# OpenResearchInstitute/ka9q-sdr

Hardware: AMD Instinct MI355X
Metric: input Msamples/s + channels @ real-time, 16384-pt overlap-save (higher is better)
Workload: dtype f32

## Files before the change

ka9q_sdr_amd/csrc/kq_pruned.hip:

```cpp
#include <cstdlib>
#include <type_traits>

#include "kq_device.hpp"
#include "kq_lane.hpp"
#include "kq_regfft.hpp"

namespace kq {

namespace {

__device__ __forceinline__ rfft::v2f as_v2f(float2 a) { return (rfft::v2f){a.x, a.y}; }
__device__ __forceinline__ float2 as_f2(rfft::v2f a) { return make_float2(a.x, a.y); }
__device__ __forceinline__ float2 cmul(float2 a, float2 b) { return as_f2(rfft::pk_cmul(as_v2f(a), as_v2f(b))); }
__device__ __forceinline__ float2 cmulc(float2 a, float2 b) { return as_f2(rfft::pk_cmul_any(as_v2f(a), as_v2f(b))); }
__device__ __forceinline__ float2 cadd(float2 a, float2 b) { return make_float2(a.x + b.x, a.y + b.y); }
__device__ __forceinline__ float2 csub(float2 a, float2 b) { return make_float2(a.x - b.x, a.y - b.y); }
__device__ __forceinline__ float2 cconj(float2 a) { return make_float2(a.x, -a.y); }
__device__ __forceinline__ float2 cfma_v(float2 b, float2 c, float2 a) { return as_f2(rfft::pk_cmadd(as_v2f(b), as_v2f(c), as_v2f(a))); }
__device__ __forceinline__ float2 cfma(float2 b, float2 c, float2 a) {
  rfft::v2f const bb = as_v2f(b), cc = as_v2f(c);
  return as_f2(rfft::pk_fma((rfft::v2f){-bb.y, bb.y}, cc.yx, rfft::pk_fma(bb.xx, cc, as_v2f(a))));
}

using rfft::bitrev5;
using rfft::kPi;
using rfft::tw_im;
using rfft::tw_re;
__device__ __forceinline__ void fft32_dit(float2 (&v)[32]) {
  rfft::v2f w[32];
#pragma unroll
  for (int i = 0; i < 32; i++) w[i] = as_v2f(v[i]);
  rfft::fft_dit_pk<32>(w);
#pragma unroll
  for (int i = 0; i < 32; i++) v[i] = as_f2(w[i]);
}

template <int ND>
struct Tab {
  static constexpr int P = ND / 32;
  static constexpr int kA = (ND == 64) ? 2 * 32 * 4 : (ND == 128) ? 32 * P * 2 : P * 32 * P * 2;
  static constexpr int kT = ND * 2;
  static constexpr int kL = 6 * ND * 2;
  static constexpr int kFloats = kA + kT + kL;
  static constexpr int kWaveF4 = (ND == 256) ? ND / 2 : (kA + kT) / 4;
};

template <int ND>
__device__ __forceinline__ int signed_bin(int q) {
  return q <= ND / 2 ? q : q - ND;
}

template <int ND>
__device__ __forceinline__ float2 table_entry_AT(int i, double f, double r, int R, int N) {
  constexpr int P = ND / 32;
  constexpr int nA = Tab<ND>::kA / 2;
  if (i < nA) {
    double a, extra = 0;
    if (ND == 64) {
      int const pass = i >> 6, ap = (i >> 1) & 31, hf = i & 1;
      a = ap + 32 * hf;
      if (pass) extra = -(double)ap / 64.0 + (hf ? 0.5 : 0.0);
    } else if (ND == 128) {
      int const ap = i / P, s = i % P;
      a = ap + 32 * s;
    } else {
      int const pass = i / (32 * P), ap = (i / P) % 32, s = i % P;
      a = ap + 32 * s;
      extra = -(double)(s * pass) / 8.0 - (double)(ap * pass) / 256.0;
    }
    double const Ra = (double)R * a;
    return phasor_turns(f * Ra + r * (0.5 * Ra * (Ra - 1.0)) + extra);
  }
  int const t = i - nA;
  int const p = t >> 5, qp = t & 31;
  int const q = P * qp + p;
  double turns = 64.0 * f;
  turns -= rint(turns);
  turns -= 64.0 * (double)signed_bin<ND>(q) / (double)N;
  return phasor_turns(turns);
}

__device__ __forceinline__ void swap32(float &a, float &b) {
  auto const r = __builtin_amdgcn_permlane32_swap(__float_as_uint(a), __float_as_uint(b), false, false);
  a = __uint_as_float(r[0]);
  b = __uint_as_float(r[1]);
}

__device__ __forceinline__ void swap16(float &a, float &b) {
  auto const r = __builtin_amdgcn_permlane16_swap(__float_as_uint(a), __float_as_uint(b), false, false);
  a = __uint_as_float(r[0]);
  b = __uint_as_float(r[1]);
}
template <int I>
__device__ __forceinline__ void pair_dpp(float &e, float &o) {
  static_assert(I == 3 || I == 2, "lane bits 3 and 2: whole banks of four lanes");
  int const ei = __float_as_int(e), oi = __float_as_int(o);
  int lo, up;
  if constexpr (I == 3) {
    lo = __builtin_amdgcn_update_dpp(ei, oi, 0x128, 0xF, 0xC, false);
    up = __builtin_amdgcn_update_dpp(oi, ei, 0x128, 0xF, 0x3, false);
  } else {
    lo = __builtin_amdgcn_update_dpp(ei, oi, 0x114, 0xF, 0xA, false);
    up = __builtin_amdgcn_update_dpp(oi, ei, 0x104, 0xF, 0x5, false);
  }
  e = __int_as_float(lo);
  o = __int_as_float(up);
}

template <int ND, int PASS, int STRIDE, bool SWEPT>
__device__ __forceinline__ void column_pass(const float2 *col, const float4 *tab, const float2 *wsh, float kappa,
                                            float2 (&v)[32]) {
  constexpr int P = ND / 32;
  constexpr int CH = (ND == 64) ? 4 : (ND == 128) ? 2 : 1;
  constexpr int TW4 = (ND == 64) ? 1 : P / 2;
  float2 xs[2][CH][P];
  float4 tw[2][CH][TW4];
#pragma unroll
  for (int i = 0; i < CH; i++) {
#pragma unroll
    for (int s = 0; s < P; s++) xs[0][i][s] = col[STRIDE * (i + 32 * s)];
#pragma unroll
    for (int t = 0; t < TW4; t++) tw[0][i][t] = (ND == 64) ? tab[PASS * 32 + i] : tab[TW4 * i + t];
  }
#pragma unroll
  for (int k = 0; k < 32 / CH; k++) {
    int const cur = k & 1, nxt = cur ^ 1;
    if (k + 1 < 32 / CH) {
#pragma unroll
      for (int i = 0; i < CH; i++) {
        int const ap = (k + 1) * CH + i;
#pragma unroll
        for (int s = 0; s < P; s++) xs[nxt][i][s] = col[STRIDE * (ap + 32 * s)];
#pragma unroll
        for (int t = 0; t < TW4; t++) tw[nxt][i][t] = (ND == 64) ? tab[PASS * 32 + ap] : tab[TW4 * ap + t];
      }
    }
    __builtin_amdgcn_sched_barrier(0);
#pragma unroll
    for (int i = 0; i < CH; i++) {
      int const ap = k * CH + i;
      float2 x[P];
#pragma unroll
      for (int s = 0; s < P; s++) {
        x[s] = xs[cur][i][s];
        if (SWEPT) {
          float const ph = kappa * (float)(ap + 32 * s);
          x[s] = make_float2(fmaf(-ph, x[s].y, x[s].x), fmaf(ph, x[s].x, x[s].y));
        }
      }
      float2 r;
      if (ND == 64) {
        float4 const t = tw[cur][i][0];
        r = make_float2(x[0].x * t.x - x[0].y * t.y, x[0].x * t.y + x[0].y * t.x);
        r.x = fmaf(x[1].x, t.z, fmaf(-x[1].y, t.w, r.x));
        r.y = fmaf(x[1].x, t.w, fmaf(x[1].y, t.z, r.y));
      } else {
        float2 re = make_float2(0.f, 0.f), ro = make_float2(0.f, 0.f);
        bool first_e = true, first_o = true;
#pragma unroll
        for (int s = 0; s < P; s++) {
          float4 const t4 = tw[cur][i][s >> 1];
          float2 const A = (s & 1) ? make_float2(t4.z, t4.w) : make_float2(t4.x, t4.y);
          int const e8 = ((8 / P) * s * PASS) & 7;
          int const rot = e8 >> 1;
          float2 const As = rot == 0   ? A
                            : rot == 1 ? make_float2(A.y, -A.x)
                            : rot == 2 ? make_float2(-A.x, -A.y)
                                       : make_float2(-A.y, A.x);
          if (e8 & 1) {
            ro = first_o ? cmulc(x[s], As) : cfma(x[s], As, ro);
            first_o = false;
          } else {
            re = first_e ? cmulc(x[s], As) : cfma(x[s], As, re);
            first_e = false;
          }
        }
        r = re;
        if (!first_o) {
          float const h = 0.70710678118654752440f;
          r.x += (ro.x + ro.y) * h;
          r.y += (ro.y - ro.x) * h;
        }
        if (PASS != 0 && ap != 0) {
          r = cmul(r, wsh[(ap * PASS) % ND]);
        }
      }
      v[bitrev5(ap)] = r;
    }
    __builtin_amdgcn_sched_barrier(0);
  }
  fft32_dit(v);
  __builtin_amdgcn_sched_barrier(0);
}

__device__ __forceinline__ void horner(float2 (&acc)[32], const float2 (&v)[32], const float4 *tT) {
#pragma unroll
  for (int k = 0; k < 4; k++) {
    float4 w4[4];
#pragma unroll
    for (int i = 0; i < 4; i++) w4[i] = tT[k * 4 + i];
#pragma unroll
    for (int i = 0; i < 4; i++) {
      int const q0 = k * 8 + 2 * i;
      acc[q0] = cfma(make_float2(w4[i].x, w4[i].y), acc[q0], v[q0]);
      acc[q0 + 1] = cfma(make_float2(w4[i].z, w4[i].w), acc[q0 + 1], v[q0 + 1]);
    }
    __builtin_amdgcn_sched_barrier(0);
  }
}

template <int ND, int PASS, bool SWEPT>
__device__ __forceinline__ float2 lane_reduce(float2 (&acc)[32], const float2 *tL, const float2 (&th)[6], int lane) {
  constexpr int P = ND / 32;
  float2 z[16];
  int qlow;
  {
    int const bit = (lane >> 5) & 1;
    qlow = bit;
    const float2 *tl = tL + 5 * ND;
#pragma unroll
    for (int m = 0; m < 16; m++) {
      float2 e = acc[2 * m], o = acc[2 * m + 1];
      swap32(e.x, o.x);
      swap32(e.y, o.y);
      float2 w = tl[P * (2 * m + bit) + PASS];
      if (SWEPT) w = cmul(w, th[5]);
      z[m] = cfma_v(w, o, e);
    }
  }
#pragma unroll
  for (int t = 1; t < 5; t++) {
    int const i = 5 - t;
    int const bit = (lane >> i) & 1;
    int const cnt = 16 >> t;
    const float2 *tl = tL + (size_t)i * ND;
#pragma unroll
    for (int m = 0; m < cnt; m++) {
      float2 lo, hi;
      if (i >= 2) {
        lo = z[2 * m];
        hi = z[2 * m + 1];
        if (i == 4) {
          swap16(lo.x, hi.x);
          swap16(lo.y, hi.y);
        } else if (i == 3) {
          pair_dpp<3>(lo.x, hi.x);
          pair_dpp<3>(lo.y, hi.y);
        } else {
          pair_dpp<2>(lo.x, hi.x);
          pair_dpp<2>(lo.y, hi.y);
        }
      } else {
        float2 const e = z[2 * m], o = z[2 * m + 1];
        float2 const keep = bit ? o : e, send = bit ? e : o;
        float2 recv;
        recv.x = __shfl_xor(send.x, 1 << i, 64);
        recv.y = __shfl_xor(send.y, 1 << i, 64);
        lo = bit ? recv : keep;
        hi = bit ? keep : recv;
      }
      int const qp = (((2 * m + bit) << t) | qlow);
      float2 w = tl[P * qp + PASS];
      if (SWEPT) w = cmul(w, th[i]);
      z[m] = cfma_v(w, hi, lo);
    }
    qlow |= bit << t;
  }
  float2 recv;
  recv.x = __shfl_xor(z[0].x, 1, 64);
  recv.y = __shfl_xor(z[0].y, 1, 64);
  int const b0 = lane & 1;
  float2 const lo = b0 ? recv : z[0], hi = b0 ? z[0] : recv;
  float2 w = tL[P * qlow + PASS];
  if (SWEPT) w = cmul(w, th[0]);
  return cfma_v(w, hi, lo);
}

template <int ND>
__device__ __forceinline__ float2 lane_reduce_rt(float2 (&acc)[32], const float2 *tL, int pass, int lane) {
  constexpr int P = ND / 32;
  float2 z[16];
  int qlow;
  {
    int const bit = (lane >> 5) & 1;
    qlow = bit;
    const float2 *tl = tL + 5 * ND + pass;
#pragma unroll
    for (int m = 0; m < 16; m++) {
      float2 e = acc[2 * m], o = acc[2 * m + 1];
      swap32(e.x, o.x);
      swap32(e.y, o.y);
      z[m] = cfma_v(tl[P * (2 * m + bit)], o, e);
    }
  }
#pragma unroll
  for (int t = 1; t < 5; t++) {
    int const i = 5 - t;
    int const bit = (lane >> i) & 1;
    int const cnt = 16 >> t;
    const float2 *tl = tL + (size_t)i * ND + pass;
#pragma unroll
    for (int m = 0; m < cnt; m++) {
      float2 lo, hi;
      if (i >= 2) {
        lo = z[2 * m];
        hi = z[2 * m + 1];
        if (i == 4) {
          swap16(lo.x, hi.x);
          swap16(lo.y, hi.y);
        } else if (i == 3) {
          pair_dpp<3>(lo.x, hi.x);
          pair_dpp<3>(lo.y, hi.y);
        } else {
          pair_dpp<2>(lo.x, hi.x);
          pair_dpp<2>(lo.y, hi.y);
        }
      } else {
        float2 const e = z[2 * m], o = z[2 * m + 1];
        float2 const keep = bit ? o : e, send = bit ? e : o;
        float2 recv;
        recv.x = __shfl_xor(send.x, 1 << i, 64);
        recv.y = __shfl_xor(send.y, 1 << i, 64);
        lo = bit ? recv : keep;
        hi = bit ? keep : recv;
      }
      int const qp = (((2 * m + bit) << t) | qlow);
      z[m] = cfma_v(tl[P * qp], hi, lo);
    }
    qlow |= bit << t;
  }
  float2 recv;
  recv.x = __shfl_xor(z[0].x, 1, 64);
  recv.y = __shfl_xor(z[0].y, 1, 64);
  int const b0 = lane & 1;
  float2 const lo = b0 ? recv : z[0], hi = b0 ? z[0] : recv;
  return cfma_v(tL[P * qlow + pass], hi, lo);
}

template <int ND, bool SWEPT>
__device__ __forceinline__ void fill_tables(float4 *wtab, const float *tc, double f_blk, double df, double r, int R, int N,
                                            float2 (&th)[6], int lane) {
  if (SWEPT) {
    float2 *w2 = reinterpret_cast<float2 *>(wtab);
    for (int i = lane; i < Tab<ND>::kWaveF4 * 2; i += 64) w2[i] = table_entry_AT<ND>(i, f_blk, r, R, N);
#pragma unroll
    for (int i = 0; i < 6; i++) th[i] = phasor_turns((double)(1 << i) * df);
  } else {
    const float4 *src = reinterpret_cast<const float4 *>(tc);
    for (int i = lane; i < Tab<ND>::kWaveF4; i += 64) wtab[i] = src[i];
#pragma unroll
    for (int i = 0; i < 6; i++) th[i] = make_float2(1.f, 0.f);
  }
  wave_sync();
}

template <int ND>
__device__ __forceinline__ void epilogue_from_scratch(const float2 *scratch, bool isb, float2 *out, int olen, int lane);

template <int ND>
__device__ __forceinline__ void epilogue_lds(float2 *scratch, const float2 (&ypass)[ND / 32], float2 p0, const float2 *H,
                                             bool isb, float2 *out, int olen, int lane) {
  constexpr int P = ND / 32, V = ND / 64;
  int const b0 = lane & 1;
  int const qp = (int)(__brev((unsigned)(lane >> 1)) >> 27);
#pragma unroll
  for (int i = 0; i < V; i++) {
    float2 const y = b0 ? ypass[2 * i + 1] : ypass[2 * i];
    int const q = P * qp + 2 * i + b0;
    scratch[q] = cmul(cmul(y, p0), H[q]);
  }
  wave_sync();
  epilogue_from_scratch<ND>(scratch, isb, out, olen, lane);
}

template <int ND>
__device__ __forceinline__ void epilogue_from_scratch(const float2 *scratch, bool isb, float2 *out, int olen, int lane) {
  constexpr int V = ND / 64;
  constexpr int LOGN = (ND == 128) ? 7 : 8, LOGV = (ND == 128) ? 1 : 2;
  float2 z[V];
#pragma unroll
  for (int e = 0; e < V; e++) {
    int const q = (int)(__brev((unsigned)(V * lane + e)) >> (32 - LOGN));
    float2 gq = scratch[q];
    if (isb && q != 0 && q != ND / 2) {
      float2 const o = scratch[ND - q];
      gq = (q < ND / 2) ? cadd(gq, cconj(o)) : csub(gq, cconj(o));
    }
    z[e] = gq;
  }
#pragma unroll
  for (int s = 0; s < LOGV; s++) {
    int const half = 1 << s;
#pragma unroll
    for (int e = 0; e < V; e++) {
      if (e & half) continue;
      int const jj = e & (half - 1);
      float2 const a = z[e];
      float2 b = z[e + half];
      if (jj != 0) b = make_float2(-b.y, b.x);
      z[e] = cadd(a, b);
      z[e + half] = csub(a, b);
    }
  }
#pragma unroll
  for (int s = LOGV; s < LOGN; s++) {
    int const half = 1 << s;
    int const bit = (lane >> (s - LOGV)) & 1;
#pragma unroll
    for (int e = 0; e < V; e++) {
      int const jj = (V * lane + e) & (half - 1);
      float sw, cw;
      sincospif((float)jj / (float)half, &sw, &cw);
      float2 const v = bit ? cmul(z[e], make_float2(cw, sw)) : z[e];
      float2 rr;
      rr.x = __shfl_xor(v.x, half / V, 64);
      rr.y = __shfl_xor(v.y, half / V, 64);
      z[e] = bit ? csub(rr, v) : cadd(v, rr);
    }
  }
  int const first = ND - olen;
#pragma unroll
  for (int e = 0; e < V; e++) {
    int const pos = V * lane + e;
    if (pos >= first) out[pos - first] = z[e];
  }
}

}

template <int ND>
__global__ void k_pruned_tables(Geom g, ChanDev ch, float *__restrict__ tab, int nchan) {
  int const c = blockIdx.x;
  if (c >= nchan) return;
  double const f = ch.lo_freq[c];
  float2 *t = reinterpret_cast<float2 *>(tab + (size_t)c * Tab<ND>::kFloats);
  constexpr int nAT = (Tab<ND>::kA + Tab<ND>::kT) / 2;
  for (int i = threadIdx.x; i < nAT; i += blockDim.x) t[i] = table_entry_AT<ND>(i, f, 0.0, g.D, g.N);
  for (int i = threadIdx.x; i < 6 * ND; i += blockDim.x) {
    int const lvl = i / ND, q = i % ND;
    double const off = (double)(1 << lvl);
    double turns = off * f;
    turns -= rint(turns);
    turns -= off * (double)signed_bin<ND>(q) / (double)g.N;
    t[nAT + i] = phasor_turns(turns);
  }
}

template <int NWAVES, int CPW, int R, bool SWEPT>
__global__ void __launch_bounds__(NWAVES * 64) k_pruned_resident(Geom g, ChanDev ch, Planes pl,
                                                                 const float2 *__restrict__ window,
                                                                 const float *__restrict__ tab, int nchan,
                                                                 const int *__restrict__ chan_list, IirArgs iir) {
  constexpr int ND = 64;
  constexpr int N = ND * R;
  constexpr int groups = R / 64;
  extern __shared__ __attribute__((aligned(16))) float2 lds[];
  int const blk = blockIdx.y;
  {
    const float4 *src = reinterpret_cast<const float4 *>(window + (size_t)blk * g.L);
    float4 *dst = reinterpret_cast<float4 *>(lds);
    for (int i = threadIdx.x; i < N / 2; i += NWAVES * 64) dst[i] = src[i];
  }
  float2 *itw = lds + N + NWAVES * Tab<ND>::kWaveF4 * 2;
  if (threadIdx.x < 32) {
    float sw, cw;
    sincospif((float)threadIdx.x / 32.f, &sw, &cw);
    itw[threadIdx.x] = make_float2(cw, sw);
  }
  __syncthreads();
  int const wave = threadIdx.x >> 6, lane = threadIdx.x & 63;
  float4 *wtab = reinterpret_cast<float4 *>(lds + N) + wave * Tab<ND>::kWaveF4;
  int const b0 = lane & 1;
  double const m0 = (double)blk * g.L;

  for (int ci = 0; ci < CPW; ci++) {
    int const idx = __builtin_amdgcn_readfirstlane((blockIdx.x * NWAVES + wave) * CPW + ci);
    if (idx >= nchan) break;
    int const c = chan_list ? __builtin_amdgcn_readfirstlane(chan_list[idx]) : idx;
    const float *tc = tab + (size_t)c * Tab<ND>::kFloats;
    const float2 *tL = reinterpret_cast<const float2 *>(tc + Tab<ND>::kA + Tab<ND>::kT);
    double const f0 = ch.lo_freq[c], r = SWEPT ? ch.lo_rate[c] : 0.0;
    double const f_blk = f0 + r * m0;
    float2 th[6];
    fill_tables<ND, SWEPT>(wtab, tc, f_blk, r * m0, r, R, N, th, lane);
    const float4 *wT = wtab + Tab<ND>::kA / 4;
    float const kap_lane = SWEPT ? (float)(2.0 * kPi * r * (double)R) : 0.f;

    float2 y_even = make_float2(0.f, 0.f), y_odd = make_float2(0.f, 0.f);
#pragma unroll
    for (int pass = 0; pass < 2; pass++) {
      float2 acc[32];
#pragma unroll 1
      for (int j = groups - 1; j >= 0; j--) {
        const float2 *col = lds + 64 * j + lane;
        float const kappa = kap_lane * (float)(64 * j + lane);
        float2 v[32];
        if (pass == 0)
          column_pass<ND, 0, R, SWEPT>(col, wtab, nullptr, kappa, v);
        else
          column_pass<ND, 1, R, SWEPT>(col, wtab, nullptr, kappa, v);
        if (j == groups - 1) {
#pragma unroll
          for (int i = 0; i < 32; i++) acc[i] = v[i];
        } else {
          horner(acc, v, wT + pass * 16);
        }
      }
      if (pass == 0)
        y_even = lane_reduce<ND, 0, SWEPT>(acc, tL, th, lane);
      else
        y_odd = lane_reduce<ND, 1, SWEPT>(acc, tL, th, lane);
    }
    float2 y = make_float2(b0 ? y_odd.x : y_even.x, b0 ? y_odd.y : y_even.y);
    int const q = (int)(__brev((unsigned)lane) >> 26);
    {
      int const src = (int)((__brev((unsigned)(q >> 1)) >> 27) << 1) | (q & 1);
      float2 t2;
      t2.x = __shfl(y.x, src, 64);
      t2.y = __shfl(y.y, src, 64);
      y = t2;
    }
    {
      double turns = ch.lo_phase[c] + f0 * m0;
      if (SWEPT) turns += r * (0.5 * m0 * (m0 - 1.0));
      y = cmul(y, phasor_turns(turns));
      y = cmul(y, ch.resp[(size_t)c * 64 + q]);
      if (ch.fflags[c] & FLAG_ISB) {
        int const qp = (64 - q) & 63;
        int const partner = (int)(__brev((unsigned)qp) >> 26);
        float2 o;
        o.x = __shfl(y.x, partner, 64);
        o.y = __shfl(y.y, partner, 64);
        if (q != 0 && q != 32) y = (q < 32) ? cadd(y, cconj(o)) : csub(y, cconj(o));
      }
    }
    auto stage = [&](auto hc) {
      constexpr int half = decltype(hc)::value;
      constexpr int sh = (half == 1) ? 5 : (half == 2) ? 4 : (half == 4) ? 3 : (half == 8) ? 2 : (half == 16) ? 1 : 0;
      bool const bit = (lane & half) != 0;
      float2 v = y;
      if (half > 1) {
        float2 const w = itw[(lane & (half - 1)) << sh];
        v = bit ? cmul(y, w) : y;
      }
      float2 rr;
      rr.x = lane_xor<half>(v.x, lane);
      rr.y = lane_xor<half>(v.y, lane);
      y = bit ? csub(rr, v) : cadd(v, rr);
    };
    stage(std::integral_constant<int, 1>{});
    stage(std::integral_constant<int, 2>{});
    stage(std::integral_constant<int, 4>{});
    stage(std::integral_constant<int, 8>{});
    stage(std::integral_constant<int, 16>{});
    stage(std::integral_constant<int, 32>{});
    int const first = 64 - g.olen;
    if (lane >= first) pl.filt[((size_t)c * g.max_blocks + blk) * g.olen + (lane - first)] = y;
  }
  if (iir.sums != nullptr && blockIdx.x == 0 && blockIdx.y == 0 && wave == NWAVES - 1)
    block_energy_iir_wave(iir.sums, iir.split, iir.update, iir.nblocks, iir.L, iir.state, iir.if_power, lane);
}

template <int NWAVES, int R, bool SWEPT>
__global__ void __launch_bounds__(NWAVES * 64) k_pruned_stream(Geom g, ChanDev ch, Planes pl,
                                                               const float2 *__restrict__ window,
                                                               const float *__restrict__ tab, int nchan,
                                                                 const int *__restrict__ chan_list) {
  constexpr int ND = 128, P = 4;
  constexpr int N = ND * R;
  constexpr int groups = R / 64;
  constexpr int kSlice = ND * 64;
  extern __shared__ __attribute__((aligned(16))) float2 lds[];
  int const blk = blockIdx.y;
  int const wave = threadIdx.x >> 6, lane = threadIdx.x & 63;
  float4 *wtab = reinterpret_cast<float4 *>(lds + 2 * kSlice) + wave * (Tab<ND>::kWaveF4 + ND / 2);
  float2 *scratch = reinterpret_cast<float2 *>(wtab + Tab<ND>::kWaveF4);
  float2 *wsh = reinterpret_cast<float2 *>(reinterpret_cast<float4 *>(lds + 2 * kSlice) + NWAVES * (Tab<ND>::kWaveF4 + ND / 2));
  for (int i = threadIdx.x; i < 128; i += NWAVES * 64) wsh[i] = phasor_turns(-(double)i / 128.0);
  const float2 *win = window + (size_t)blk * g.L;
  double const m0 = (double)blk * g.L;

  int const idx = __builtin_amdgcn_readfirstlane(min((int)(blockIdx.x * NWAVES + wave), nchan - 1));
  int const c = chan_list ? __builtin_amdgcn_readfirstlane(chan_list[idx]) : idx;
  bool const live = (int)(blockIdx.x * NWAVES + wave) < nchan;
  const float *tc = tab + (size_t)c * Tab<ND>::kFloats;
  const float2 *tL = reinterpret_cast<const float2 *>(tc + Tab<ND>::kA + Tab<ND>::kT);
  double const f0 = ch.lo_freq[c], r = SWEPT ? ch.lo_rate[c] : 0.0;
  double const f_blk = f0 + r * m0;
  float2 th[6];
  fill_tables<ND, SWEPT>(wtab, tc, f_blk, r * m0, r, R, N, th, lane);
  const float4 *wT = wtab + Tab<ND>::kA / 4;
  float const kap_lane = SWEPT ? (float)(2.0 * kPi * r * (double)R) : 0.f;

  unsigned const lane_off = (unsigned)(lane >> 5) * (unsigned)(R * sizeof(float2)) + (unsigned)(lane & 31) * 16u;
  auto stage = [&](int j, int buf) {
    constexpr int rows_per_wave = ND / NWAVES;
    const char *slice0 = reinterpret_cast<const char *>(win + (size_t)(wave * rows_per_wave) * R + 64 * j);
#pragma unroll
    for (int i = 0; i < rows_per_wave / 2; i++) {
      const char *ubase = slice0 + (size_t)(2 * i) * R * sizeof(float2);
      float2 *dst = lds + buf * kSlice + (wave * rows_per_wave + 2 * i) * 64;
      __builtin_amdgcn_global_load_lds(ubase + lane_off, (__attribute__((address_space(3))) void *)dst, 16, 0, 0);
    }
  };

  float2 ypass[P];
  int step = 0;
  stage(groups - 1, 0);
  auto do_pass = [&](auto pass_c) {
    constexpr int pass = decltype(pass_c)::value;
    float2 acc[32];
#pragma unroll 1
    for (int j = groups - 1; j >= 0; j--, step++) {
      asm volatile("s_waitcnt vmcnt(0)" ::: "memory");
      __syncthreads();
      if (j > 0)
        stage(j - 1, (step + 1) & 1);
      else if (pass + 1 < P)
        stage(groups - 1, (step + 1) & 1);
      const float2 *col = lds + (step & 1) * kSlice + lane;
      float const kappa = kap_lane * (float)(64 * j + lane);
      float2 v[32];
      column_pass<ND, pass, 64, SWEPT>(col, wtab, wsh, kappa, v);
      if (j == groups - 1) {
#pragma unroll
        for (int i = 0; i < 32; i++) acc[i] = v[i];
      } else {
        horner(acc, v, wT + pass * 16);
      }
    }
    ypass[pass] = lane_reduce<ND, pass, SWEPT>(acc, tL, th, lane);
  };
  do_pass(std::integral_constant<int, 0>{});
  do_pass(std::integral_constant<int, 1>{});
  do_pass(std::integral_constant<int, 2>{});
  do_pass(std::integral_constant<int, 3>{});
  if (!live) return;
  {
    double turns = ch.lo_phase[c] + f0 * m0;
    if (SWEPT) turns += r * (0.5 * m0 * (m0 - 1.0));
    epilogue_lds<ND>(scratch, ypass, phasor_turns(turns), ch.resp + (size_t)c * ND, (ch.fflags[c] & FLAG_ISB) != 0,
                     pl.filt + ((size_t)c * g.max_blocks + blk) * g.olen, g.olen, lane);
  }
}

template <int NWAVES, int CPW>
__global__ void __launch_bounds__(NWAVES * 64) k_pruned_resident256(Geom g, ChanDev ch, Planes pl,
                                                                    const float2 *__restrict__ window,
                                                                    const float *__restrict__ tab, int nchan,
                                                                 const int *__restrict__ chan_list) {
  constexpr int ND = 256, P = 8, R = 64;
  constexpr int N = ND * R;
  extern __shared__ __attribute__((aligned(16))) float2 lds[];
  int const blk = blockIdx.y;
  {
    const float4 *src = reinterpret_cast<const float4 *>(window + (size_t)blk * g.L);
    float4 *dst = reinterpret_cast<float4 *>(lds);
    for (int i = threadIdx.x; i < N / 2; i += NWAVES * 64) dst[i] = src[i];
  }
  __syncthreads();
  int const wave = threadIdx.x >> 6, lane = threadIdx.x & 63;
  float2 *scratch = lds + N + wave * ND;
  double const m0 = (double)blk * g.L;
  int const vzero = __builtin_amdgcn_mbcnt_lo(0u, 0u);
  int const b0 = lane & 1;
  int const qp = (int)(__brev((unsigned)(lane >> 1)) >> 27);
  float2 th[6];
#pragma unroll
  for (int i = 0; i < 6; i++) th[i] = make_float2(1.f, 0.f);

  for (int ci = 0; ci < CPW; ci++) {
    int const idx = __builtin_amdgcn_readfirstlane((blockIdx.x * NWAVES + wave) * CPW + ci);
    if (idx >= nchan) break;
    int const c = chan_list ? __builtin_amdgcn_readfirstlane(chan_list[idx]) : idx;
    const float *tc = tab + (size_t)c * Tab<ND>::kFloats;
    const float2 *tL = reinterpret_cast<const float2 *>(tc + Tab<ND>::kA + Tab<ND>::kT);
    const float2 *H = ch.resp + (size_t)c * ND;
    float2 const p0 = phasor_turns(ch.lo_phase[c] + ch.lo_freq[c] * m0);
    const float2 *col = lds + lane;
#pragma unroll 1
    for (int pass = 0; pass < P; pass++) {
      const float4 *tp = reinterpret_cast<const float4 *>(tc) + (size_t)pass * 32 * 4 + vzero;
      float2 v[32];
      float2 xs[2][P];
      float4 tw[2][4];
#pragma unroll
      for (int s = 0; s < P; s++) xs[0][s] = col[R * (32 * s)];
#pragma unroll
      for (int t = 0; t < 4; t++) tw[0][t] = tp[t];
#pragma unroll
      for (int ap = 0; ap < 32; ap++) {
        int const cur = ap & 1, nxt = cur ^ 1;
        if (ap + 1 < 32) {
#pragma unroll
          for (int s = 0; s < P; s++) xs[nxt][s] = col[R * (ap + 1 + 32 * s)];
#pragma unroll
          for (int t = 0; t < 4; t++) tw[nxt][t] = tp[4 * (ap + 1) + t];
        }
        __builtin_amdgcn_sched_barrier(0);
        float2 r = cmul(xs[cur][0], make_float2(tw[cur][0].x, tw[cur][0].y));
        r = cfma(xs[cur][1], make_float2(tw[cur][0].z, tw[cur][0].w), r);
#pragma unroll
        for (int t = 1; t < 4; t++) {
          r = cfma(xs[cur][2 * t], make_float2(tw[cur][t].x, tw[cur][t].y), r);
          r = cfma(xs[cur][2 * t + 1], make_float2(tw[cur][t].z, tw[cur][t].w), r);
        }
        v[bitrev5(ap)] = r;
        __builtin_amdgcn_sched_barrier(0);
      }
      fft32_dit(v);
      __builtin_amdgcn_sched_barrier(0);
      float2 const y = lane_reduce_rt<ND>(v, tL, pass, lane);
      if (b0 == (pass & 1)) {
        int const q = P * qp + pass;
        scratch[q] = cmul(cmul(y, p0), H[q]);
      }
    }
    wave_sync();
    epilogue_from_scratch<ND>(scratch, (ch.fflags[c] & FLAG_ISB) != 0, pl.filt + ((size_t)c * g.max_blocks + blk) * g.olen,
                              g.olen, lane);
    wave_sync();
  }
}

bool pruned_supported(const Geom &g) {
  if (g.Ndec == 64) return g.D == 64 || g.D == 128 || g.D == 256;
  if (g.Ndec == 256) return g.D == 64;
  return g.Ndec == 128 && g.D == 512;
}
size_t pruned_table_elems(const Geom &g) {
  return (size_t)(g.Ndec == 64 ? Tab<64>::kFloats : g.Ndec == 128 ? Tab<128>::kFloats : Tab<256>::kFloats) / 2;
}

void launch_pruned_tables(hipStream_t s, const Geom &g, const ChanDev &ch, float2 *chan_tw, int nchan) {
  if (g.Ndec == 64)
    hipLaunchKernelGGL(k_pruned_tables<64>, dim3(nchan), dim3(256), 0, s, g, ch, reinterpret_cast<float *>(chan_tw), nchan);
  else if (g.Ndec == 128)
    hipLaunchKernelGGL(k_pruned_tables<128>, dim3(nchan), dim3(256), 0, s, g, ch, reinterpret_cast<float *>(chan_tw), nchan);
  else
    hipLaunchKernelGGL(k_pruned_tables<256>, dim3(nchan), dim3(256), 0, s, g, ch, reinterpret_cast<float *>(chan_tw), nchan);
}

namespace {
template <int R, bool SWEPT>
void launch_resident(hipStream_t s, const Geom &g, const ChanDev &ch, const Planes &pl, const float2 *window, const float *tab,
                     int nchan, int nblocks, const int *chan_list, const IirArgs &iir) {
  constexpr int NWAVES = 8, CPW = 4;
  size_t const lds_bytes = (size_t)64 * R * sizeof(float2) + (size_t)NWAVES * Tab<64>::kWaveF4 * sizeof(float4) +
                           32 * sizeof(float2);
  ensure_dynamic_lds((const void *)k_pruned_resident<NWAVES, CPW, R, SWEPT>, (size_t)(lds_bytes));
  int const per_wg = NWAVES * CPW;
  hipLaunchKernelGGL((k_pruned_resident<NWAVES, CPW, R, SWEPT>), dim3((nchan + per_wg - 1) / per_wg, nblocks),
                     dim3(NWAVES * 64), lds_bytes, s, g, ch, pl, window, tab, nchan, chan_list, iir);
}

void launch_resident256(hipStream_t s, const Geom &g, const ChanDev &ch, const Planes &pl, const float2 *window,
                        const float *tab, int nchan, int nblocks, const int *chan_list) {
  constexpr int NWAVES = 8, CPW = 4;
  size_t const lds_bytes = (size_t)16384 * sizeof(float2) + (size_t)NWAVES * 256 * sizeof(float2);
  ensure_dynamic_lds((const void *)k_pruned_resident256<NWAVES, CPW>, (size_t)(lds_bytes));
  int const per_wg = NWAVES * CPW;
  hipLaunchKernelGGL((k_pruned_resident256<NWAVES, CPW>), dim3((nchan + per_wg - 1) / per_wg, nblocks),
                     dim3(NWAVES * 64), lds_bytes, s, g, ch, pl, window, tab, nchan, chan_list);
}

template <bool SWEPT>
void launch_stream(hipStream_t s, const Geom &g, const ChanDev &ch, const Planes &pl, const float2 *window, const float *tab,
                   int nchan, int nblocks, const int *chan_list) {
  constexpr int NWAVES = 8, R = 512;
  size_t const lds_bytes = (size_t)2 * 128 * 64 * sizeof(float2) + (size_t)NWAVES * (Tab<128>::kWaveF4 + 64) * sizeof(float4) +
                           128 * sizeof(float2);
  ensure_dynamic_lds((const void *)k_pruned_stream<NWAVES, R, SWEPT>, (size_t)(lds_bytes));
  hipLaunchKernelGGL((k_pruned_stream<NWAVES, R, SWEPT>), dim3((nchan + NWAVES - 1) / NWAVES, nblocks), dim3(NWAVES * 64),
                     lds_bytes, s, g, ch, pl, window, tab, nchan, chan_list);
}
}

bool pruned_carries_iir(const Geom &g) { return g.Ndec == 64 && (g.D == 256 || g.D == 128 || g.D == 64); }

void launch_filter_pruned(hipStream_t s, const Geom &g, const ChanDev &ch, const Planes &pl, const float2 *window,
                          const float2 *chan_tw, int nchan, int nblocks, bool swept, const int *chan_list, const IirArgs &iir) {
  const float *tab = reinterpret_cast<const float *>(chan_tw);
  if (g.Ndec == 256) {
    launch_resident256(s, g, ch, pl, window, tab, nchan, nblocks, chan_list);
    return;
  }
  if (g.Ndec == 128) {
    if (swept)
      launch_stream<true>(s, g, ch, pl, window, tab, nchan, nblocks, chan_list);
    else
      launch_stream<false>(s, g, ch, pl, window, tab, nchan, nblocks, chan_list);
    return;
  }
#define KQ_RES(RR)                                                           \
  if (g.D == RR) {                                                           \
    if (swept)                                                               \
      launch_resident<RR, true>(s, g, ch, pl, window, tab, nchan, nblocks, chan_list, iir);  \
    else                                                                     \
      launch_resident<RR, false>(s, g, ch, pl, window, tab, nchan, nblocks, chan_list, iir); \
    return;                                                                  \
  }
  KQ_RES(256)
  KQ_RES(128)
  KQ_RES(64)
#undef KQ_RES
}

}
```

Before: 375,900.

## Switch pruned FFT kernels to packed v2f math with inline-asm premultiply

Converts the pruned overlap-save kernels from float2 to the packed v2f vector type throughout (column pass, horner, lane reduce), so the compiler emits v_pk_fma/v_pk_mul more consistently. It adds a hand-written inline-asm packed premultiply for the ND=64 path and folds the runtime-pass lane_reduce_rt into the templated lane_reduce. It also splits the ND=64 LDS column base into two pointers so the upper row offset stays within the DS instruction immediate range. This is meant to cut VALU instruction count and address arithmetic, at the cost of relying on hand-encoded op_sel/neg modifiers being correct.

```diff
diff --git a/ka9q_sdr_amd/csrc/kq_pruned.hip b/ka9q_sdr_amd/csrc/kq_pruned.hip
--- a/ka9q_sdr_amd/csrc/kq_pruned.hip
+++ b/ka9q_sdr_amd/csrc/kq_pruned.hip
@@ -9,31 +9,42 @@
 
 namespace {
 
-__device__ __forceinline__ rfft::v2f as_v2f(float2 a) { return (rfft::v2f){a.x, a.y}; }
-__device__ __forceinline__ float2 as_f2(rfft::v2f a) { return make_float2(a.x, a.y); }
+using rfft::v2f;
+__device__ __forceinline__ v2f as_v2f(float2 a) { return (v2f){a.x, a.y}; }
+__device__ __forceinline__ float2 as_f2(v2f a) { return make_float2(a.x, a.y); }
+__device__ __forceinline__ v2f lo2(float4 a) { return (v2f){a.x, a.y}; }
+__device__ __forceinline__ v2f hi2(float4 a) { return (v2f){a.z, a.w}; }
+__device__ __forceinline__ v2f cmul(v2f a, v2f b) { return rfft::pk_cmul(a, b); }
 __device__ __forceinline__ float2 cmul(float2 a, float2 b) { return as_f2(rfft::pk_cmul(as_v2f(a), as_v2f(b))); }
-__device__ __forceinline__ float2 cmulc(float2 a, float2 b) { return as_f2(rfft::pk_cmul_any(as_v2f(a), as_v2f(b))); }
+__device__ __forceinline__ v2f cmulc(v2f a, v2f b) { return rfft::pk_cmul_any(a, b); }
 __device__ __forceinline__ float2 cadd(float2 a, float2 b) { return make_float2(a.x + b.x, a.y + b.y); }
 __device__ __forceinline__ float2 csub(float2 a, float2 b) { return make_float2(a.x - b.x, a.y - b.y); }
 __device__ __forceinline__ float2 cconj(float2 a) { return make_float2(a.x, -a.y); }
-__device__ __forceinline__ float2 cfma_v(float2 b, float2 c, float2 a) { return as_f2(rfft::pk_cmadd(as_v2f(b), as_v2f(c), as_v2f(a))); }
-__device__ __forceinline__ float2 cfma(float2 b, float2 c, float2 a) {
-  rfft::v2f const bb = as_v2f(b), cc = as_v2f(c);
-  return as_f2(rfft::pk_fma((rfft::v2f){-bb.y, bb.y}, cc.yx, rfft::pk_fma(bb.xx, cc, as_v2f(a))));
+__device__ __forceinline__ v2f cfma_v(v2f b, v2f c, v2f a) { return rfft::pk_cmadd(b, c, a); }
+__device__ __forceinline__ v2f cfma(v2f b, v2f c, v2f a) {
+  return rfft::pk_fma((v2f){-b.y, b.y}, c.yx, rfft::pk_fma(b.xx, c, a));
+}
+
+__device__ __forceinline__ v2f premul2(v2f x0, v2f a0, v2f x1, v2f a1) {
+  v2f m, r0, r1, r2;
+  asm("v_pk_mul_f32 %0, %1, %2 op_sel:[1,1] op_sel_hi:[1,0]" : "=v"(m) : "v"(x0), "v"(a0));
+  asm("v_pk_fma_f32 %0, %1, %2, %3 op_sel_hi:[0,1,1] neg_lo:[0,0,1]" : "=v"(r0) : "v"(x0), "v"(a0), "v"(m));
+  asm("v_pk_fma_f32 %0, %1, %2, %3 op_sel:[1,1,0] op_sel_hi:[1,0,1] neg_lo:[1,0,0]" : "=v"(r1) : "v"(x1), "v"(a1), "v"(r0));
+  asm("v_pk_fma_f32 %0, %1, %2, %3 op_sel_hi:[0,1,1]" : "=v"(r2) : "v"(x1), "v"(a1), "v"(r1));
+  return r2;
+}
+__device__ __forceinline__ v2f premul2c(v2f x0, v2f a0, v2f x1, v2f a1) {
+  v2f const m = x0.yy * a0.yx;
+  v2f r = rfft::pk_fma(x0.xx, a0, (v2f){-m.x, m.y});
+  r = rfft::pk_fma((v2f){-x1.y, x1.y}, a1.yx, r);
+  return rfft::pk_fma(x1.xx, a1, r);
 }
 
 using rfft::bitrev5;
 using rfft::kPi;
 using rfft::tw_im;
 using rfft::tw_re;
-__device__ __forceinline__ void fft32_dit(float2 (&v)[32]) {
-  rfft::v2f w[32];
-#pragma unroll
-  for (int i = 0; i < 32; i++) w[i] = as_v2f(v[i]);
-  rfft::fft_dit_pk<32>(w);
-#pragma unroll
-  for (int i = 0; i < 32; i++) v[i] = as_f2(w[i]);
-}
+__device__ __forceinline__ void fft32_dit(v2f (&v)[32]) { rfft::fft_dit_pk<32>(v); }
 
 template <int ND>
 struct Tab {
@@ -80,19 +91,21 @@
   return phasor_turns(turns);
 }
 
-__device__ __forceinline__ void swap32(float &a, float &b) {
-  auto const r = __builtin_amdgcn_permlane32_swap(__float_as_uint(a), __float_as_uint(b), false, false);
-  a = __uint_as_float(r[0]);
-  b = __uint_as_float(r[1]);
-}
-
-__device__ __forceinline__ void swap16(float &a, float &b) {
-  auto const r = __builtin_amdgcn_permlane16_swap(__float_as_uint(a), __float_as_uint(b), false, false);
-  a = __uint_as_float(r[0]);
-  b = __uint_as_float(r[1]);
+__device__ __forceinline__ void swap32(v2f &a, v2f &b) {
+  auto const rx = __builtin_amdgcn_permlane32_swap(__float_as_uint(a.x), __float_as_uint(b.x), false, false);
+  auto const ry = __builtin_amdgcn_permlane32_swap(__float_as_uint(a.y), __float_as_uint(b.y), false, false);
+  a = (v2f){__uint_as_float(rx[0]), __uint_as_float(ry[0])};
+  b = (v2f){__uint_as_float(rx[1]), __uint_as_float(ry[1])};
+}
+
+__device__ __forceinline__ void swap16(v2f &a, v2f &b) {
+  auto const rx = __builtin_amdgcn_permlane16_swap(__float_as_uint(a.x), __float_as_uint(b.x), false, false);
+  auto const ry = __builtin_amdgcn_permlane16_swap(__float_as_uint(a.y), __float_as_uint(b.y), false, false);
+  a = (v2f){__uint_as_float(rx[0]), __uint_as_float(ry[0])};
+  b = (v2f){__uint_as_float(rx[1]), __uint_as_float(ry[1])};
 }
 template <int I>
-__device__ __forceinline__ void pair_dpp(float &e, float &o) {
+__device__ __forceinline__ void pair_dpp1(float &e, float &o) {
   static_assert(I == 3 || I == 2, "lane bits 3 and 2: whole banks of four lanes");
   int const ei = __float_as_int(e), oi = __float_as_int(o);
   int lo, up;
@@ -106,19 +119,36 @@
   e = __int_as_float(lo);
   o = __int_as_float(up);
 }
+template <int I>
+__device__ __forceinline__ void pair_dpp(v2f &e, v2f &o) {
+  float ex = e.x, ey = e.y, ox = o.x, oy = o.y;
+  pair_dpp1<I>(ex, ox);
+  pair_dpp1<I>(ey, oy);
+  e = (v2f){ex, ey};
+  o = (v2f){ox, oy};
+}
+template <int I>
+__device__ __forceinline__ void pair_sel(v2f &e, v2f &o, bool bit, int lane) {
+  static_assert(I == 1 || I == 0, "lane bits 1 and 0");
+  v2f const keep = bit ? o : e, send = bit ? e : o;
+  v2f const recv = (v2f){lane_xor<1 << I>(send.x, lane), lane_xor<1 << I>(send.y, lane)};
+  e = bit ? recv : keep;
+  o = bit ? keep : recv;
+}
 
 template <int ND, int PASS, int STRIDE, bool SWEPT>
-__device__ __forceinline__ void column_pass(const float2 *col, const float4 *tab, const float2 *wsh, float kappa,
-                                            float2 (&v)[32]) {
+__device__ __forceinline__ void column_pass(const float2 *col, const float2 *colh, const float4 *tab, const float2 *wsh,
+                                            float kappa, v2f (&v)[32]) {
   constexpr int P = ND / 32;
   constexpr int CH = (ND == 64) ? 4 : (ND == 128) ? 2 : 1;
   constexpr int TW4 = (ND == 64) ? 1 : P / 2;
+  auto row = [&](int ap, int s) { return (ND == 64 && s == 1) ? colh[STRIDE * ap] : col[STRIDE * (ap + 32 * s)]; };
   float2 xs[2][CH][P];
   float4 tw[2][CH][TW4];
 #pragma unroll
   for (int i = 0; i < CH; i++) {
 #pragma unroll
-    for (int s = 0; s < P; s++) xs[0][i][s] = col[STRIDE * (i + 32 * s)];
+    for (int s = 0; s < P; s++) xs[0][i][s] = row(i, s);
 #pragma unroll
     for (int t = 0; t < TW4; t++) tw[0][i][t] = (ND == 64) ? tab[PASS * 32 + i] : tab[TW4 * i + t];
   }
@@ -130,7 +160,7 @@
       for (int i = 0; i < CH; i++) {
         int const ap = (k + 1) * CH + i;
 #pragma unroll
-        for (int s = 0; s < P; s++) xs[nxt][i][s] = col[STRIDE * (ap + 32 * s)];
+        for (int s = 0; s < P; s++) xs[nxt][i][s] = row(ap, s);
 #pragma unroll
         for (int t = 0; t < TW4; t++) tw[nxt][i][t] = (ND == 64) ? tab[PASS * 32 + ap] : tab[TW4 * ap + t];
       }
@@ -139,34 +169,32 @@
 #pragma unroll
     for (int i = 0; i < CH; i++) {
       int const ap = k * CH + i;
-      float2 x[P];
+      v2f x[P];
 #pragma unroll
       for (int s = 0; s < P; s++) {
-        x[s] = xs[cur][i][s];
+        x[s] = as_v2f(xs[cur][i][s]);
         if (SWEPT) {
           float const ph = kappa * (float)(ap + 32 * s);
-          x[s] = make_float2(fmaf(-ph, x[s].y, x[s].x), fmaf(ph, x[s].x, x[s].y));
+          x[s] = (v2f){fmaf(-ph, x[s].y, x[s].x), fmaf(ph, x[s].x, x[s].y)};
         }
       }
-      float2 r;
+      v2f r;
       if (ND == 64) {
         float4 const t = tw[cur][i][0];
-        r = make_float2(x[0].x * t.x - x[0].y * t.y, x[0].x * t.y + x[0].y * t.x);
-        r.x = fmaf(x[1].x, t.z, fmaf(-x[1].y, t.w, r.x));
-        r.y = fmaf(x[1].x, t.w, fmaf(x[1].y, t.z, r.y));
+        r = (SWEPT && STRIDE == 64) ? premul2c(x[0], lo2(t), x[1], hi2(t)) : premul2(x[0], lo2(t), x[1], hi2(t));
       } else {
-        float2 re = make_float2(0.f, 0.f), ro = make_float2(0.f, 0.f);
+        v2f re = (v2f){0.f, 0.f}, ro = (v2f){0.f, 0.f};
         bool first_e = true, first_o = true;
 #pragma unroll
         for (int s = 0; s < P; s++) {
           float4 const t4 = tw[cur][i][s >> 1];
-          float2 const A = (s & 1) ? make_float2(t4.z, t4.w) : make_float2(t4.x, t4.y);
+          v2f const A = (s & 1) ? hi2(t4) : lo2(t4);
           int const e8 = ((8 / P) * s * PASS) & 7;
           int const rot = e8 >> 1;
-          float2 const As = rot == 0   ? A
-                            : rot == 1 ? make_float2(A.y, -A.x)
-                            : rot == 2 ? make_float2(-A.x, -A.y)
-                                       : make_float2(-A.y, A.x);
+          v2f const As = rot == 0   ? A
+                         : rot == 1 ? (v2f){A.y, -A.x}
+                         : rot == 2 ? (v2f){-A.x, -A.y}
+                                    : (v2f){-A.y, A.x};
           if (e8 & 1) {
             ro = first_o ? cmulc(x[s], As) : cfma(x[s], As, ro);
             first_o = false;
@@ -182,7 +210,7 @@
           r.y += (ro.y - ro.x) * h;
         }
         if (PASS != 0 && ap != 0) {
-          r = cmul(r, wsh[(ap * PASS) % ND]);
+          r = cmul(r, as_v2f(wsh[(ap * PASS) % ND]));
         }
       }
       v[bitrev5(ap)] = r;
@@ -193,7 +221,7 @@
   __builtin_amdgcn_sched_barrier(0);
 }
 
-__device__ __forceinline__ void horner(float2 (&acc)[32], const float2 (&v)[32], const float4 *tT) {
+__device__ __forceinline__ void horner(v2f (&acc)[32], const v2f (&v)[32], const float4 *tT) {
 #pragma unroll
   for (int k = 0; k < 4; k++) {
     float4 w4[4];
@@ -202,17 +230,19 @@
 #pragma unroll
     for (int i = 0; i < 4; i++) {
       int const q0 = k * 8 + 2 * i;
-      acc[q0] = cfma(make_float2(w4[i].x, w4[i].y), acc[q0], v[q0]);
-      acc[q0 + 1] = cfma(make_float2(w4[i].z, w4[i].w), acc[q0 + 1], v[q0 + 1]);
+      acc[q0] = cfma_v(lo2(w4[i]), acc[q0], v[q0]);
+      acc[q0 + 1] = cfma_v(hi2(w4[i]), acc[q0 + 1], v[q0 + 1]);
     }
     __builtin_amdgcn_sched_barrier(0);
   }
 }
 
 template <int ND, int PASS, bool SWEPT>
-__device__ __forceinline__ float2 lane_reduce(float2 (&acc)[32], const float2 *tL, const float2 (&th)[6], int lane) {
+__device__ __forceinline__ v2f lane_reduce(v2f (&acc)[32], const float2 *tL, const v2f (&th)[6], int lane, int pass = PASS) {
   constexpr int P = ND / 32;
-  float2 z[16];
+  static_assert(PASS >= 0 || !SWEPT, "the run-time pass is unswept");
+  tL += (PASS < 0) ? pass : PASS;
+  v2f z[16];
   int qlow;
   {
     int const bit = (lane >> 5) & 1;
@@ -220,10 +250,9 @@
     const float2 *tl = tL + 5 * ND;
 #pragma unroll
     for (int m = 0; m < 16; m++) {
-      float2 e = acc[2 * m], o = acc[2 * m + 1];
-      swap32(e.x, o.x);
-      swap32(e.y, o.y);
-      float2 w = tl[P * (2 * m + bit) + PASS];
+      v2f e = acc[2 * m], o = acc[2 * m + 1];
+      swap32(e, o);
+      v2f w = as_v2f(tl[P * (2 * m + bit)]);
       if (SWEPT) w = cmul(w, th[5]);
       z[m] = cfma_v(w, o, e);
     }
@@ -236,120 +265,43 @@
     const float2 *tl = tL + (size_t)i * ND;
 #pragma unroll
     for (int m = 0; m < cnt; m++) {
-      float2 lo, hi;
-      if (i >= 2) {
-        lo = z[2 * m];
-        hi = z[2 * m + 1];
-        if (i == 4) {
-          swap16(lo.x, hi.x);
-          swap16(lo.y, hi.y);
-        } else if (i == 3) {
-          pair_dpp<3>(lo.x, hi.x);
-          pair_dpp<3>(lo.y, hi.y);
-        } else {
-          pair_dpp<2>(lo.x, hi.x);
-          pair_dpp<2>(lo.y, hi.y);
-        }
-      } else {
-        float2 const e = z[2 * m], o = z[2 * m + 1];
-        float2 const keep = bit ? o : e, send = bit ? e : o;
-        float2 recv;
-        recv.x = __shfl_xor(send.x, 1 << i, 64);
-        recv.y = __shfl_xor(send.y, 1 << i, 64);
-        lo = bit ? recv : keep;
-        hi = bit ? keep : recv;
-      }
+      v2f lo = z[2 * m], hi = z[2 * m + 1];
+      if (i == 4)
+        swap16(lo, hi);
+      else if (i == 3)
+        pair_dpp<3>(lo, hi);
+      else if (i == 2)
+        pair_dpp<2>(lo, hi);
+      else
+        pair_sel<1>(lo, hi, bit != 0, lane);
       int const qp = (((2 * m + bit) << t) | qlow);
-      float2 w = tl[P * qp + PASS];
+      v2f w = as_v2f(tl[P * qp]);
       if (SWEPT) w = cmul(w, th[i]);
       z[m] = cfma_v(w, hi, lo);
     }
     qlow |= bit << t;
   }
-  float2 recv;
-  recv.x = __shfl_xor(z[0].x, 1, 64);
-  recv.y = __shfl_xor(z[0].y, 1, 64);
-  int const b0 = lane & 1;
-  float2 const lo = b0 ? recv : z[0], hi = b0 ? z[0] : recv;
-  float2 w = tL[P * qlow + PASS];
+  v2f const recv = (v2f){lane_xor<1>(z[0].x, lane), lane_xor<1>(z[0].y, lane)};
+  bool const b0 = (lane & 1) != 0;
+  v2f const lo = b0 ? recv : z[0], hi = b0 ? z[0] : recv;
+  v2f w = as_v2f(tL[P * qlow]);
   if (SWEPT) w = cmul(w, th[0]);
   return cfma_v(w, hi, lo);
 }
 
-template <int ND>
-__device__ __forceinline__ float2 lane_reduce_rt(float2 (&acc)[32], const float2 *tL, int pass, int lane) {
-  constexpr int P = ND / 32;
-  float2 z[16];
-  int qlow;
-  {
-    int const bit = (lane >> 5) & 1;
-    qlow = bit;
-    const float2 *tl = tL + 5 * ND + pass;
-#pragma unroll
-    for (int m = 0; m < 16; m++) {
-      float2 e = acc[2 * m], o = acc[2 * m + 1];
-      swap32(e.x, o.x);
-      swap32(e.y, o.y);
-      z[m] = cfma_v(tl[P * (2 * m + bit)], o, e);
-    }
-  }
-#pragma unroll
-  for (int t = 1; t < 5; t++) {
-    int const i = 5 - t;
-    int const bit = (lane >> i) & 1;
-    int const cnt = 16 >> t;
-    const float2 *tl = tL + (size_t)i * ND + pass;
-#pragma unroll
-    for (int m = 0; m < cnt; m++) {
-      float2 lo, hi;
-      if (i >= 2) {
-        lo = z[2 * m];
-        hi = z[2 * m + 1];
-        if (i == 4) {
-          swap16(lo.x, hi.x);
-          swap16(lo.y, hi.y);
-        } else if (i == 3) {
-          pair_dpp<3>(lo.x, hi.x);
-          pair_dpp<3>(lo.y, hi.y);
-        } else {
-          pair_dpp<2>(lo.x, hi.x);
-          pair_dpp<2>(lo.y, hi.y);
-        }
-      } else {
-        float2 const e = z[2 * m], o = z[2 * m + 1];
-        float2 const keep = bit ? o : e, send = bit ? e : o;
-        float2 recv;
-        recv.x = __shfl_xor(send.x, 1 << i, 64);
-        recv.y = __shfl_xor(send.y, 1 << i, 64);
-        lo = bit ? recv : keep;
-        hi = bit ? keep : recv;
-      }
-      int const qp = (((2 * m + bit) << t) | qlow);
-      z[m] = cfma_v(tl[P * qp], hi, lo);
-    }
-    qlow |= bit << t;
-  }
-  float2 recv;
-  recv.x = __shfl_xor(z[0].x, 1, 64);
-  recv.y = __shfl_xor(z[0].y, 1, 64);
-  int const b0 = lane & 1;
-  float2 const lo = b0 ? recv : z[0], hi = b0 ? z[0] : recv;
-  return cfma_v(tL[P * qlow + pass], hi, lo);
-}
-
 template <int ND, bool SWEPT>
 __device__ __forceinline__ void fill_tables(float4 *wtab, const float *tc, double f_blk, double df, double r, int R, int N,
-                                            float2 (&th)[6], int lane) {
+                                            v2f (&th)[6], int lane) {
   if (SWEPT) {
     float2 *w2 = reinterpret_cast<float2 *>(wtab);
     for (int i = lane; i < Tab<ND>::kWaveF4 * 2; i += 64) w2[i] = table_entry_AT<ND>(i, f_blk, r, R, N);
 #pragma unroll
-    for (int i = 0; i < 6; i++) th[i] = phasor_turns((double)(1 << i) * df);
+    for (int i = 0; i < 6; i++) th[i] = as_v2f(phasor_turns((double)(1 << i) * df));
   } else {
     const float4 *src = reinterpret_cast<const float4 *>(tc);
     for (int i = lane; i < Tab<ND>::kWaveF4; i += 64) wtab[i] = src[i];
 #pragma unroll
-    for (int i = 0; i < 6; i++) th[i] = make_float2(1.f, 0.f);
+    for (int i = 0; i < 6; i++) th[i] = (v2f){1.f, 0.f};
   }
   wave_sync();
 }
@@ -358,14 +310,14 @@
 __device__ __forceinline__ void epilogue_from_scratch(const float2 *scratch, bool isb, float2 *out, int olen, int lane);
 
 template <int ND>
-__device__ __forceinline__ void epilogue_lds(float2 *scratch, const float2 (&ypass)[ND / 32], float2 p0, const float2 *H,
+__device__ __forceinline__ void epilogue_lds(float2 *scratch, const v2f (&ypass)[ND / 32], float2 p0, const float2 *H,
                                              bool isb, float2 *out, int olen, int lane) {
   constexpr int P = ND / 32, V = ND / 64;
   int const b0 = lane & 1;
   int const qp = (int)(__brev((unsigned)(lane >> 1)) >> 27);
 #pragma unroll
   for (int i = 0; i < V; i++) {
-    float2 const y = b0 ? ypass[2 * i + 1] : ypass[2 * i];
+    float2 const y = as_f2(b0 ? ypass[2 * i + 1] : ypass[2 * i]);
     int const q = P * qp + 2 * i + b0;
     scratch[q] = cmul(cmul(y, p0), H[q]);
   }
@@ -454,6 +406,7 @@
   constexpr int ND = 64;
   constexpr int N = ND * R;
   constexpr int groups = R / 64;
+  constexpr bool kSplitBase = (size_t)63 * R * sizeof(float2) > 65535;
   extern __shared__ __attribute__((aligned(16))) float2 lds[];
   int const blk = blockIdx.y;
   {
@@ -481,24 +434,27 @@
     const float2 *tL = reinterpret_cast<const float2 *>(tc + Tab<ND>::kA + Tab<ND>::kT);
     double const f0 = ch.lo_freq[c], r = SWEPT ? ch.lo_rate[c] : 0.0;
     double const f_blk = f0 + r * m0;
-    float2 th[6];
+    v2f th[6];
     fill_tables<ND, SWEPT>(wtab, tc, f_blk, r * m0, r, R, N, th, lane);
     const float4 *wT = wtab + Tab<ND>::kA / 4;
     float const kap_lane = SWEPT ? (float)(2.0 * kPi * r * (double)R) : 0.f;
 
-    float2 y_even = make_float2(0.f, 0.f), y_odd = make_float2(0.f, 0.f);
+    v2f y_even = (v2f){0.f, 0.f}, y_odd = (v2f){0.f, 0.f};
 #pragma unroll
     for (int pass = 0; pass < 2; pass++) {
-      float2 acc[32];
+      v2f acc[32];
 #pragma unroll 1
       for (int j = groups - 1; j >= 0; j--) {
-        const float2 *col = lds + 64 * j + lane;
-        float const kappa = kap_lane * (float)(64 * j + lane);
-        float2 v[32];
+        int const b = 64 * j + lane;
+        int bh = b + 32 * R;
+        if (kSplitBase) asm("" : "+v"(bh));
+        const float2 *col = lds + b, *colh = lds + bh;
+        float const kappa = kap_lane * (float)b;
+        v2f v[32];
         if (pass == 0)
-          column_pass<ND, 0, R, SWEPT>(col, wtab, nullptr, kappa, v);
+          column_pass<ND, 0, R, SWEPT>(col, colh, wtab, nullptr, kappa, v);
         else
-          column_pass<ND, 1, R, SWEPT>(col, wtab, nullptr, kappa, v);
+          column_pass<ND, 1, R, SWEPT>(col, colh, wtab, nullptr, kappa, v);
         if (j == groups - 1) {
 #pragma unroll
           for (int i = 0; i < 32; i++) acc[i] = v[i];
@@ -511,7 +467,7 @@
       else
         y_odd = lane_reduce<ND, 1, SWEPT>(acc, tL, th, lane);
     }
-    float2 y = make_float2(b0 ? y_odd.x : y_even.x, b0 ? y_odd.y : y_even.y);
+    float2 y = as_f2(b0 ? y_odd : y_even);
     int const q = (int)(__brev((unsigned)lane) >> 26);
     {
       int const src = (int)((__brev((unsigned)(q >> 1)) >> 27) << 1) | (q & 1);
@@ -587,7 +543,7 @@
   const float2 *tL = reinterpret_cast<const float2 *>(tc + Tab<ND>::kA + Tab<ND>::kT);
   double const f0 = ch.lo_freq[c], r = SWEPT ? ch.lo_rate[c] : 0.0;
   double const f_blk = f0 + r * m0;
-  float2 th[6];
+  v2f th[6];
   fill_tables<ND, SWEPT>(wtab, tc, f_blk, r * m0, r, R, N, th, lane);
   const float4 *wT = wtab + Tab<ND>::kA / 4;
   float const kap_lane = SWEPT ? (float)(2.0 * kPi * r * (double)R) : 0.f;
@@ -604,12 +560,12 @@
     }
   };
 
-  float2 ypass[P];
+  v2f ypass[P];
   int step = 0;
   stage(groups - 1, 0);
   auto do_pass = [&](auto pass_c) {
     constexpr int pass = decltype(pass_c)::value;
-    float2 acc[32];
+    v2f acc[32];
 #pragma unroll 1
     for (int j = groups - 1; j >= 0; j--, step++) {
       asm volatile("s_waitcnt vmcnt(0)" ::: "memory");
@@ -620,8 +576,8 @@
         stage(groups - 1, (step + 1) & 1);
       const float2 *col = lds + (step & 1) * kSlice + lane;
       float const kappa = kap_lane * (float)(64 * j + lane);
-      float2 v[32];
-      column_pass<ND, pass, 64, SWEPT>(col, wtab, wsh, kappa, v);
+      v2f v[32];
+      column_pass<ND, pass, 64, SWEPT>(col, nullptr, wtab, wsh, kappa, v);
       if (j == groups - 1) {
 #pragma unroll
         for (int i = 0; i < 32; i++) acc[i] = v[i];
@@ -665,9 +621,9 @@
   int const vzero = __builtin_amdgcn_mbcnt_lo(0u, 0u);
   int const b0 = lane & 1;
   int const qp = (int)(__brev((unsigned)(lane >> 1)) >> 27);
-  float2 th[6];
-#pragma unroll
-  for (int i = 0; i < 6; i++) th[i] = make_float2(1.f, 0.f);
+  v2f th[6];
+#pragma unroll
+  for (int i = 0; i < 6; i++) th[i] = (v2f){1.f, 0.f};
 
   for (int ci = 0; ci < CPW; ci++) {
     int const idx = __builtin_amdgcn_readfirstlane((blockIdx.x * NWAVES + wave) * CPW + ci);
@@ -681,7 +637,7 @@
 #pragma unroll 1
     for (int pass = 0; pass < P; pass++) {
       const float4 *tp = reinterpret_cast<const float4 *>(tc) + (size_t)pass * 32 * 4 + vzero;
-      float2 v[32];
+      v2f v[32];
       float2 xs[2][P];
       float4 tw[2][4];
 #pragma unroll
@@ -698,19 +654,19 @@
           for (int t = 0; t < 4; t++) tw[nxt][t] = tp[4 * (ap + 1) + t];
         }
         __builtin_amdgcn_sched_barrier(0);
-        float2 r = cmul(xs[cur][0], make_float2(tw[cur][0].x, tw[cur][0].y));
-        r = cfma(xs[cur][1], make_float2(tw[cur][0].z, tw[cur][0].w), r);
+        v2f r = cmul(as_v2f(xs[cur][0]), lo2(tw[cur][0]));
+        r = cfma_v(as_v2f(xs[cur][1]), hi2(tw[cur][0]), r);
 #pragma unroll
         for (int t = 1; t < 4; t++) {
-          r = cfma(xs[cur][2 * t], make_float2(tw[cur][t].x, tw[cur][t].y), r);
-          r = cfma(xs[cur][2 * t + 1], make_float2(tw[cur][t].z, tw[cur][t].w), r);
+          r = cfma_v(as_v2f(xs[cur][2 * t]), lo2(tw[cur][t]), r);
+          r = cfma_v(as_v2f(xs[cur][2 * t + 1]), hi2(tw[cur][t]), r);
         }
         v[bitrev5(ap)] = r;
         __builtin_amdgcn_sched_barrier(0);
       }
       fft32_dit(v);
       __builtin_amdgcn_sched_barrier(0);
-      float2 const y = lane_reduce_rt<ND>(v, tL, pass, lane);
+      float2 const y = as_f2(lane_reduce<ND, -1, false>(v, tL, th, lane, pass));
       if (b0 == (pass & 1)) {
         int const q = P * qp + pass;
         scratch[q] = cmul(cmul(y, p0), H[q]);
```

Result: no change. 375,800 (-0.0%).
